# martinruenz/maskfusion

Hardware: NVIDIA H100
Metric: frames/sec on 640x480 .klg replay (higher is better)
Workload: dtype f32

## Files before the change

maskfusion_b200/csrc/mf_track.cu:

```cuda
#include "mf_common.cuh"
#include "mf_kernels.h"
#include "mf_host.h"
#include <float.h>
#include <algorithm>
#include <stdlib.h>
#include <string>

namespace mfb {

#ifndef MFB200_DEFAULT_TRACK_CACHE
#define MFB200_DEFAULT_TRACK_CACHE 0
#endif
#define CACHE_BYTES_PER_SLOT 44
#define TRK_THREADS 256
#define NACC_ICP 29
#define NACC_RGB 27
#define NACC (NACC_ICP + NACC_RGB)

MF_D float3 m3v(const float* R, float3 v)
{
    return make_float3((R[0] * v.x + R[1] * v.y) + R[2] * v.z, (R[3] * v.x + R[4] * v.y) + R[5] * v.z, (R[6] * v.x + R[7] * v.y) + R[8] * v.z);
}

__device__ void ldltSolve(const double* Ain, const double* b, int n, double* x)
// ... 245 lines not shown
{
    __shared__ bool isLast;
    __threadfence();
    __syncthreads();
    if (threadIdx.x == 0) {
        unsigned t = atomicAdd(ticket, 1u);
        isLast = (t == gridDim.x - 1);
        if (isLast) *ticket = 0;
    }
    __syncthreads();
    if (isLast) __threadfence();
    return isLast;
}

__global__ void __launch_bounds__(TRK_THREADS) k_icp_only(const float4* __restrict__ vmapC, const float4* __restrict__ nmapC,
                                                          const float4* __restrict__ vmapG, const float4* __restrict__ nmapG,
                                                          int W, int H, Cam cam, TrackPoses pp, float distThres, float angleThres,
                                                          double* __restrict__ partial, unsigned* ticket, float* out29)
{
    double acc[NACC_ICP];
#pragma unroll
    for (int k = 0; k < NACC_ICP; ++k) acc[k] = 0.0;
    const float* Rc = pp.p[0]; const float* tc = pp.p[0] + 9; const float* Rpi = pp.p[1]; const float* tp = pp.p[1] + 9;
    const float3 tprev = make_float3(tp[0], tp[1], tp[2]);
    const int N = W * H;
    for (int i = blockIdx.x * blockDim.x + threadIdx.x; i < N; i += gridDim.x * blockDim.x) {
        float4 vc4 = vmapC[i];
        float3 vg = m3v(Rc, make_float3(vc4.x, vc4.y, vc4.z));
        vg = make_float3(vg.x + tc[0], vg.y + tc[1], vg.z + tc[2]);
        float3 vcp = m3v(Rpi, sub3(vg, tprev));
        int ux = __float2int_rn(vcp.x * cam.fx / vcp.z + cam.cx);
        int uy = __float2int_rn(vcp.y * cam.fy / vcp.z + cam.cy);
        if (ux < 0 || uy < 0 || ux >= W || uy >= H || vcp.z < 0) continue;
        int j = uy * W + ux;
        float4 vp4 = __ldg(vmapG + j), np4 = __ldg(nmapG + j), nc4 = nmapC[i];
        float3 vp = make_float3(vp4.x, vp4.y, vp4.z), np_ = make_float3(np4.x, np4.y, np4.z);
        float3 ng = m3v(Rc, make_float3(nc4.x, nc4.y, nc4.z));
        float3 d = sub3(vp, vg);
        float dist = sqrtf((d.x * d.x + d.y * d.y) + d.z * d.z);
        float3 c = cross3(ng, np_);
        float sine = sqrtf((c.x * c.x + c.y * c.y) + c.z * c.z);
        if (!(sine < angleThres && dist <= distThres && !isnan(nc4.x) && !isnan(np4.x))) continue;
        float3 s_cp = vcp, d_cp = m3v(Rpi, sub3(vp, tprev)), n_cp = m3v(Rpi, np_);
        float row[7];
        row[0] = n_cp.x; row[1] = n_cp.y; row[2] = n_cp.z;
        row[3] = s_cp.y * n_cp.z - s_cp.z * n_cp.y;
        row[4] = s_cp.z * n_cp.x - s_cp.x * n_cp.z;
        row[5] = s_cp.x * n_cp.y - s_cp.y * n_cp.x;
        row[6] = (n_cp.x * (s_cp.x - d_cp.x) + n_cp.y * (s_cp.y - d_cp.y)) + n_cp.z * (s_cp.z - d_cp.z);
        int q = 0;
#pragma unroll
        for (int a = 0; a < 6; ++a)
#pragma unroll
            for (int b = a; b < 7; ++b) { acc[q] = fma((double)row[a], (double)row[b], acc[q]); ++q; }
        acc[27] = fma((double)row[6], (double)row[6], acc[27]);
        acc[28] += 1.0;
    }
    blockReduceStore<NACC_ICP>(acc, partial + (size_t)blockIdx.x * 32);
    if (!lastBlock(ticket)) return;
    __shared__ double tot[NACC_ICP];
    sumPartials<NACC_ICP>(partial, gridDim.x, tot);
    if (threadIdx.x < NACC_ICP) out29[threadIdx.x] = (float)tot[threadIdx.x];
}

#ifndef PT_THREADS
#define PT_THREADS 512
#endif
#define PT_WARPS (PT_THREADS / 32)
#define ROWF 32

struct TrackParams {
    int W, H; Cam cam;
    int icp, rgb, rgbOnly, so3;
    int iterations[3];
    float icpWeight, angleThres, distThres, sobelScale, maxDepthDelta;
    float minScale[3];
    int corrSlots;
    int bitWords;
    int cacheRounds;
    unsigned llBase;
    int nJobs; unsigned short jobStart[TRACK_MAX_JOBS + 1];
};

MF_D double shflXorD(double v, int m)
{
    return __hiloint2double(__shfl_xor_sync(0xffffffffu, __double2hiint(v), m), __shfl_xor_sync(0xffffffffu, __double2loint(v), m));
}
template <int H>
MF_D void warpHalvingStep(double* v, int lane)
{
    const bool up = (lane & H) != 0;
#pragma unroll
    for (int k = 0; k < H; ++k) {
        double keep = up ? v[k + H] : v[k];
        double send = up ? v[k] : v[k + H];
        v[k] = keep + shflXorD(send, H);
    }
}
MF_D void warpReduceHalving32(double* v)
{
    const int lane = threadIdx.x & 31;
    warpHalvingStep<16>(v, lane);
    warpHalvingStep<8>(v, lane);
    warpHalvingStep<4>(v, lane);
    warpHalvingStep<2>(v, lane);
    warpHalvingStep<1>(v, lane);
}

MF_D void llStore(uint4* p, double v, unsigned flag)
{
    asm volatile("st.volatile.global.v4.u32 [%0], {%1, %2, %3, %4};" ::"l"(p), "r"((unsigned)__double2loint(v)), "r"(flag), "r"((unsigned)__double2hiint(v)), "r"(flag) : "memory");
}
MF_D uint4 llLoad(const uint4* p)
{
    uint4 r;
    asm volatile("ld.volatile.global.v4.u32 {%0, %1, %2, %3}, [%4];" : "=r"(r.x), "=r"(r.y), "=r"(r.z), "=r"(r.w) : "l"(p) : "memory");
    return r;
}

template <int N>
MF_D void ctaReduceStore(const double* acc, double (*red)[ROWF], uint4* __restrict__ rowOut, unsigned flag, int extra0, int extra1)
{
    double v[32];
#pragma unroll
    for (int k = 0; k < 32; ++k) v[k] = k < N ? acc[k] : 0.0;
    v[29] = (double)extra0; v[30] = (double)extra1;
    warpReduceHalving32(v);
    const int lane = threadIdx.x & 31, warp = threadIdx.x >> 5;
    red[warp][lane] = v[0];
    __syncthreads();
    if (threadIdx.x < ROWF) {
        double s = 0;
#pragma unroll
        for (int w = 0; w < PT_WARPS; ++w) s += red[w][threadIdx.x];
        llStore(rowOut + threadIdx.x, s, flag);
    }
}
#define SUM_BATCH 10
MF_D void sumRows(const uint4* __restrict__ rows, unsigned R, unsigned flag, double (*ws)[ROWF], double* tot)
{
    const int lane = threadIdx.x & 31, warp = threadIdx.x >> 5;
    double a0 = 0;
    for (unsigned base = warp; base < R; base += PT_WARPS * SUM_BATCH) {
        uint4 x[SUM_BATCH];
        unsigned pending = 0;
#pragma unroll
        for (int i = 0; i < SUM_BATCH; ++i) { x[i] = make_uint4(0, 0, 0, 0); if (base + (unsigned)i * PT_WARPS < R) pending |= 1u << i; }
        while (pending) {
#pragma unroll
            for (int i = 0; i < SUM_BATCH; ++i)
                if ((pending >> i) & 1u) x[i] = llLoad(rows + (size_t)(base + (unsigned)i * PT_WARPS) * ROWF + lane);
#pragma unroll
            for (int i = 0; i < SUM_BATCH; ++i)
                if ((pending >> i) & 1u) { if (__all_sync(0xffffffffu, x[i].y == flag && x[i].w == flag)) pending &= ~(1u << i); }
        }
#pragma unroll
        for (int i = 0; i < SUM_BATCH; ++i) a0 += __hiloint2double((int)x[i].z, (int)x[i].x);
    }
    ws[warp][lane] = a0;
    __syncthreads();
    if (threadIdx.x < ROWF) {
        double s2 = 0;
#pragma unroll
        for (int w = 0; w < PT_WARPS; ++w) s2 += ws[w][threadIdx.x];
        tot[threadIdx.x] = s2;
    }
    __syncthreads();
}

struct RedCtx { uint4* rows; unsigned G, Gact, gen, llBase, bx; };
template <int N>
MF_D void reduceStep(const double* acc, int e0, int e1, bool active, RedCtx& rc, double (*red)[ROWF], double (*ws)[ROWF], double* tot)
{
    uint4* rows = rc.rows + (size_t)(rc.gen & 1) * rc.G * ROWF;
    ++rc.gen;
    const unsigned flag = rc.llBase + rc.gen;
    if (active) ctaReduceStore<N>(acc, red, rows + (size_t)rc.bx * ROWF, flag, e0, e1);
    sumRows(rows, rc.Gact, flag, ws, tot);
}

MF_D void gradU8(const uint8_t* __restrict__ img, int W, int x, int y, float& gx, float& gy)
{
    float actu = img[y * W + x], back = img[y * W + x - 1], fore = img[y * W + x + 1];
    gx = ((back + actu) / 2.0f) - ((fore + actu) / 2.0f);
    back = img[(y - 1) * W + x]; fore = img[(y + 1) * W + x];
    gy = ((back + actu) / 2.0f) - ((fore + actu) / 2.0f);
}


template <int LD>
MF_D double inv3dEntry(const double* M, int e)
{
    const int r = e / 3, c = e - 3 * r;
    const int c1 = c == 2 ? 0 : c + 1, c2 = c1 == 2 ? 0 : c1 + 1, r1 = r == 2 ? 0 : r + 1, r2 = r1 == 2 ? 0 : r1 + 1;
    const double cof = M[c1 * LD + r1] * M[c2 * LD + r2] - M[c1 * LD + r2] * M[c2 * LD + r1];
    const double c00 = M[LD + 1] * M[2 * LD + 2] - M[LD + 2] * M[2 * LD + 1], c01 = M[LD + 2] * M[2 * LD] - M[LD] * M[2 * LD + 2],
                 c02 = M[LD] * M[2 * LD + 1] - M[LD + 1] * M[2 * LD];
    const double det = M[0] * c00 + M[1] * c01 + M[2] * c02;
    return cof * (1.0 / det);
}

#ifdef MF_TRACK_TIMING
__device__ long long g_trackTiming[8192];
__device__ int g_trackTimingN;
#define TT(tag) do { if (blockIdx.x == 0 && threadIdx.x == 0) { int q_ = g_trackTimingN; if (q_ + 2 <= 8192) { g_trackTiming[q_] = (tag); g_trackTiming[q_ + 1] = clock64(); g_trackTimingN = q_ + 2; } } } while (0)
#else
#define TT(tag) do { } while (0)
#endif

struct SolveScratch { double A[36], b[6], x[6], Rt[16], nr[16], Ri[9], K[9], Kinv[9], tmp[9], ti[3]; float trR[9], trT[3], iR[9], iT[3]; int fast; };

MF_D void computeWarpCoop(TrackState* st, Cam c, SolveScratch* sc, int lane)
{
    const double* T = st->resultRt;
    const double* K = sc->K;
    if (lane < 9) sc->Ri[lane] = inv3dEntry<4>(T, lane);
    __syncwarp();
    if (lane < 3) sc->ti[lane] = -(sc->Ri[lane * 3] * T[3] + sc->Ri[lane * 3 + 1] * T[7] + sc->Ri[lane * 3 + 2] * T[11]);
    if (lane < 9) { int r = lane / 3, cc = lane % 3; sc->tmp[lane] = K[r * 3] * sc->Ri[cc] + K[r * 3 + 1] * sc->Ri[3 + cc] + K[r * 3 + 2] * sc->Ri[6 + cc]; }
    __syncwarp();
    if (lane < 9) { int r = lane / 3, cc = lane % 3; st->krk[lane] = (float)(sc->tmp[r * 3] * sc->Kinv[cc] + sc->tmp[r * 3 + 1] * sc->Kinv[3 + cc] + sc->tmp[r * 3 + 2] * sc->Kinv[6 + cc]); }
    if (lane < 3) st->kt[lane] = (float)(K[lane * 3] * sc->ti[0] + K[lane * 3 + 1] * sc->ti[1] + K[lane * 3 + 2] * sc->ti[2]);
    __syncwarp();
}

__device__ __noinline__ void solveAndUpdate(TrackState* st, const double* tot, bool ICP, bool RGB, float icpWeight, Cam cam, SolveScratch* sc)
{
    const int lane = threadIdx.x & 31;
    const double wgt = icpWeight;
    const int r6 = lane < 6 ? lane : 5;
    double arow[6], bown;
    {
        auto comb = [&](int c2, bool isA) -> double {
            const int a = r6 < c2 ? r6 : c2, b = r6 < c2 ? c2 : r6;
            const int q = 7 * a - (a * (a - 1)) / 2 + (b - a);
            const float vi = (float)tot[q], vr = (float)tot[NACC_ICP + q];
            if (ICP && RGB) return isA ? (double)vr + wgt * wgt * (double)vi : (double)vr + wgt * (double)vi;
            if (ICP) return (double)vi;
            return (double)vr;
        };
#pragma unroll
        for (int j = 0; j < 6; ++j) arow[j] = comb(j, true);
        bown = comb(6, false);
        if (lane < 6) {
#pragma unroll
            for (int j = 0; j < 6; ++j) st->lastA[lane * 6 + j] = arow[j];
            st->lastb[lane] = bown;
        }
    }
    if (ICP && lane == 31) { st->lastICPError = sqrtf((float)tot[27]) / (float)tot[28]; st->lastICPCount = (float)tot[28]; }
    TT(20);
    ldltSolvePivWarpRegs<6>(arow, bown, sc->x);
    TT(21);
    {
        double rx = sc->x[3], ry = sc->x[4], rz = sc->x[5];
        const double theta = sqrt(rx * rx + ry * ry + rz * rz);
        double c = 1.0, s = 0.0, c1 = 0.0;
        const bool rot = theta >= DBL_EPSILON;
        if (rot) { detSincos(theta, &s, &c); c1 = 1. - c; const double it = 1. / theta; rx *= it; ry *= it; rz *= it; }
        if (lane < 16) {
            const int r = lane >> 2, cc = lane & 3;
            double v;
            if (r == 3) v = cc == 3 ? 1.0 : 0.0;
            else if (cc == 3) v = sc->x[r];
            else if (!rot) v = r == cc ? 1.0 : 0.0;
            else {
                const double ur = r == 0 ? rx : r == 1 ? ry : rz, uc = cc == 0 ? rx : cc == 1 ? ry : rz;
                const double rrt = ur * uc;
                const int d = cc - r;
                const int o = 3 - r - cc;
                const double uo = o == 0 ? rx : o == 1 ? ry : rz;
                const double rxm = (r == cc) ? 0.0 : ((d == 1 || d == -2) ? -uo : uo);
                v = c * (r == cc ? 1.0 : 0.0) + c1 * rrt + s * rxm;
            }
            sc->Rt[lane] = v;
        }
    }
    __syncwarp();
    TT(22);
    if (lane < 16) {
        const int r = lane >> 2, c = lane & 3;
        double s2 = 0;
#pragma unroll
        for (int k = 0; k < 4; ++k) s2 += sc->Rt[r * 4 + k] * st->resultRt[k * 4 + c];
        sc->nr[lane] = s2;
    }
    __syncwarp();
    const double* T = sc->nr;
    if (lane < 16) st->resultRt[lane] = T[lane];
    if (lane < 9) st->trR[lane] = (float)T[(lane / 3) * 4 + lane % 3];
    else if (lane < 12) st->trT[lane - 9] = (float)T[(lane - 9) * 4 + 3];
    if (lane < 9) {
        const int r = lane / 3, c = lane % 3;
        const float i0 = (float)T[c * 4 + 0], i1 = (float)T[c * 4 + 1], i2 = (float)T[c * 4 + 2];
        st->Rcurr[lane] = (st->Rprev[r * 3] * i0 + st->Rprev[r * 3 + 1] * i1) + st->Rprev[r * 3 + 2] * i2;
    } else if (lane < 12) {
        const int r = lane - 9;
        const float t0 = (float)T[3], t1 = (float)T[7], t2 = (float)T[11];
        float iT[3];
#pragma unroll
        for (int k = 0; k < 3; ++k) iT[k] = -(((float)T[0 * 4 + k] * t0 + (float)T[1 * 4 + k] * t1) + (float)T[2 * 4 + k] * t2);
        st->tcurr[r] = ((st->Rprev[r * 3] * iT[0] + st->Rprev[r * 3 + 1] * iT[1]) + st->Rprev[r * 3 + 2] * iT[2]) + st->tprev[r];
    }
    TT(23);
    if (RGB && lane >= 16 && lane < 28) {
        const double* K = sc->K;
        double Ri[9];
#pragma unroll
        for (int e = 0; e < 9; ++e) Ri[e] = inv3dEntry<4>(T, e);
        const int l = lane - 16;
        if (l < 9) {
            const int r = l / 3, cc = l % 3;
            double tmp[3];
#pragma unroll
            for (int j = 0; j < 3; ++j) tmp[j] = K[r * 3] * Ri[j] + K[r * 3 + 1] * Ri[3 + j] + K[r * 3 + 2] * Ri[6 + j];
            st->krk[l] = (float)(tmp[0] * sc->Kinv[cc] + tmp[1] * sc->Kinv[3 + cc] + tmp[2] * sc->Kinv[6 + cc]);
        } else {
            const int q = l - 9;
            double ti[3];
#pragma unroll
            for (int j = 0; j < 3; ++j) ti[j] = -(Ri[j * 3] * T[3] + Ri[j * 3 + 1] * T[7] + Ri[j * 3 + 2] * T[11]);
            st->kt[q] = (float)(K[q * 3] * ti[0] + K[q * 3 + 1] * ti[1] + K[q * 3 + 2] * ti[2]);
        }
    }
}

MF_D void prefetchL1(const void* p) { asm volatile("prefetch.global.L1 [%0];" ::"l"(p)); }

struct PixA {
    float4 vc, nc; float d1; int valid, ni, x, y;
    bool rOK, iOK; int jr, ji, u0, v0; float td1; float3 vg, vcp;
    float d0; int li; float4 vp4, np4;
};

extern __shared__ int2 corrShared[];

__global__ void __launch_bounds__(PT_THREADS, 1) k_track_persistent(const TrackJob* __restrict__ jobs, TrackParams tp)
{
    __shared__ TrackJob J;
    __shared__ TrackState S;
    __shared__ SolveScratch sc;
    __shared__ double red[PT_WARPS][ROWF];
    __shared__ double ws[PT_WARPS][ROWF];
    __shared__ double tot[64];
    __shared__ double totR[ROWF];
    __shared__ float so3B[9], so3Kinv[9], so3Krlr[9];
    __shared__ double so3K[9], so3KinvD[9];
    __shared__ int flag;
    unsigned job = 0;
    while ((int)job + 1 < tp.nJobs && blockIdx.x >= tp.jobStart[job + 1]) ++job;
    const unsigned bx = blockIdx.x - tp.jobStart[job];
    const unsigned G = (unsigned)tp.jobStart[job + 1] - tp.jobStart[job];
    {
        const uint32_t* src = reinterpret_cast<const uint32_t*>(jobs + job);
        uint32_t* dst = reinterpret_cast<uint32_t*>(&J);
        for (int k = threadIdx.x; k < (int)(sizeof(TrackJob) / 4); k += PT_THREADS) dst[k] = src[k];
    }
    TrackState* st = &S;
#ifdef MF_TRACK_TIMING
    if (blockIdx.x == 0 && threadIdx.x == 0) g_trackTimingN = 0;
#endif
    TT(1);
    __syncthreads();
    if (threadIdx.x == 0) {
        const float* P = J.dpose->pose.m;
        for (int r = 0; r < 3; ++r) { for (int c = 0; c < 3; ++c) st->Rprev[r * 3 + c] = P[r * 4 + c]; st->tprev[r] = P[r * 4 + 3]; }
        for (int k = 0; k < 9; ++k) st->Rcurr[k] = st->Rprev[k];
        for (int k = 0; k < 3; ++k) st->tcurr[k] = st->tprev[k];
        inv3f(st->Rprev, st->RprevInv);
        for (int k = 0; k < 16; ++k) st->resultRt[k] = (k % 5 == 0) ? 1.0 : 0.0;
        for (int k = 0; k < 9; ++k) { st->resultR[k] = (k % 4 == 0) ? 1.0 : 0.0; st->lastResultR[k] = st->resultR[k]; st->R_lr[k] = (k % 4 == 0) ? 1.f : 0.f; st->trR[k] = (k % 4 == 0) ? 1.f : 0.f; }
        st->trT[0] = st->trT[1] = st->trT[2] = 0;
        st->so3LastError = FLT_MAX / 2; st->so3LastCount = FLT_MAX / 2; st->so3Done = 0;
        st->levelBreak = 0; st->lastRGBError = FLT_MAX; st->lastRGBCount = 0; st->lastICPError = 0; st->lastICPCount = 0;
        st->lastSO3Error = 0; st->lastSO3Count = 0; st->sigmaVal = 0;
        for (int k = 0; k < 36; ++k) st->lastA[k] = 0;
        for (int k = 0; k < 6; ++k) st->lastb[k] = 0;
    }
    __syncthreads();
    RedCtx rc;
    rc.rows = reinterpret_cast<uint4*>(J.partial); rc.G = G; rc.Gact = G; rc.gen = 0; rc.llBase = tp.llBase; rc.bx = bx;
    const size_t corrNeed = (size_t)((tp.W * tp.H + G * PT_THREADS - 1) / (G * PT_THREADS)) * PT_THREADS;
    int2* const corr = ((size_t)tp.corrSlots >= corrNeed && tp.corrSlots) ? corrShared : reinterpret_cast<int2*>(J.corres[0]) + (size_t)bx * corrNeed;
    const int cacheSlots = tp.cacheRounds * PT_THREADS;
    unsigned char* const cacheBase = reinterpret_cast<unsigned char*>(corrShared) + (((size_t)tp.corrSlots * sizeof(int2) + 15) & ~(size_t)15);
    float4* const vcS = reinterpret_cast<float4*>(cacheBase);
    float4* const ncS = vcS + cacheSlots;
    float* const d1S = reinterpret_cast<float*>(ncS + cacheSlots);
    uint32_t* const pkS = reinterpret_cast<uint32_t*>(d1S + cacheSlots);
    uint32_t* const gS = pkS + cacheSlots;
    uint32_t* const bitsS = gS + cacheSlots;

    if (tp.so3) {
        const int W = tp.W >> 2, H = tp.H >> 2, N = W * H;
        const unsigned Gact = min(G, (unsigned)((N + PT_THREADS - 1) / PT_THREADS));
        const bool active = bx < Gact;
        const int tid = (int)bx * PT_THREADS + threadIdx.x, nthr = (int)Gact * PT_THREADS;
        const Cam c = camLevel(tp.cam, 2);
        const uint8_t* __restrict__ lastImage = J.lastNextImage2;
        const uint8_t* __restrict__ nextImage = J.nextImage[2];
        if (threadIdx.x == 0) {
            double K[9] = {c.fx, 0, c.cx, 0, c.fy, c.cy, 0, 0, 1}, Kinv[9];
            inv3d(K, Kinv);
            for (int q = 0; q < 9; ++q) { so3K[q] = K[q]; so3KinvD[q] = Kinv[q]; so3Kinv[q] = (float)Kinv[q]; }
        }
        __syncthreads();
        for (int it = 0; it < 10; ++it) {
            if (threadIdx.x < 9) {
                const int r = threadIdx.x / 3, cc = threadIdx.x % 3;
                double kr[3];
#pragma unroll
                for (int q = 0; q < 3; ++q) kr[q] = so3K[r * 3] * st->resultR[q] + so3K[r * 3 + 1] * st->resultR[3 + q] + so3K[r * 3 + 2] * st->resultR[6 + q];
                so3Krlr[threadIdx.x] = (float)(cc == 0 ? kr[0] : cc == 1 ? kr[1] : kr[2]);
                so3B[threadIdx.x] = (float)(kr[0] * so3KinvD[cc] + kr[1] * so3KinvD[3 + cc] + kr[2] * so3KinvD[6 + cc]);
            }
            __syncthreads();
            TT(11);
            double acc[11];
#pragma unroll
            for (int k = 0; k < 11; ++k) acc[k] = 0;
            if (active) {
                for (int k = tid; k < N; k += nthr) {
                    int y = k / W, x = k - y * W;
                    float3 ur = make_float3((float)x, (float)y, 1.0f);
                    float3 wr = m3v(so3B, ur);
                    int wx = __float2int_rn(wr.x / wr.z), wy = __float2int_rn(wr.y / wr.z);
                    bool found = (wx >= 1 && wx < W - 1 && wy >= 1 && wy < H - 1 && x >= 1 && x < W - 1 && y >= 1 && y < H - 1);
                    if (found) {
                        float gnx, gny, glx, gly;
                        gradU8(nextImage, W, wx, wy, gnx, gny);
                        gradU8(lastImage, W, x, y, glx, gly);
                        float gx = (gnx + glx) / 2.0f, gy = (gny + gly) / 2.0f;
                        float3 p = m3v(so3Kinv, ur);
                        float z2 = p.z * p.z;
                        float a = so3Krlr[0], b = so3Krlr[1], cc = so3Krlr[2], d = so3Krlr[3], e = so3Krlr[4], f = so3Krlr[5], g = so3Krlr[6], h = so3Krlr[7], i = so3Krlr[8];
                        float fy = (float)y, fxx = (float)x;
                        float3 l = make_float3(((p.z * (d * gy + a * gx)) - (gy * g * fy) - (gx * g * fxx)) / z2,
                                               ((p.z * (e * gy + b * gx)) - (gy * h * fy) - (gx * h * fxx)) / z2,
                                               ((p.z * (f * gy + cc * gx)) - (gy * i * fy) - (gx * i * fxx)) / z2);
                        float row[4];
                        row[0] = l.y * p.z - l.z * p.y;
                        row[1] = l.z * p.x - l.x * p.z;
                        row[2] = l.x * p.y - l.y * p.x;
                        row[3] = -((float)nextImage[wy * W + wx] - (float)lastImage[k]);
                        int q = 0;
#pragma unroll
                        for (int ii = 0; ii < 3; ++ii)
#pragma unroll
                            for (int jj = ii; jj < 4; ++jj) { acc[q] = fma((double)row[ii], (double)row[jj], acc[q]); ++q; }
                        acc[9] = fma((double)row[3], (double)row[3], acc[9]);
                        acc[10] += 1.0;
                    }
                }
            }
            TT(12);
            rc.Gact = Gact;
            reduceStep<11>(acc, 0, 0, active, rc, red, ws, tot);
            TT(15);
            if (threadIdx.x < 32) {
                int mode = 0;
                if (threadIdx.x == 0) {
                    float res0 = (float)tot[9], res1 = (float)tot[10];
                    st->lastSO3Error = sqrtf(res0) / res1; st->lastSO3Count = res1;
                    if (st->lastSO3Error < st->so3LastError && fabsf(st->so3LastError - st->lastSO3Count) < 0.001f) mode = 0;
                    else if (st->lastSO3Error > st->so3LastError + 0.001f) {
                        st->lastSO3Error = st->so3LastError; st->lastSO3Count = st->so3LastCount;
                        for (int q = 0; q < 9; ++q) st->resultR[q] = st->lastResultR[q];
                        mode = 1;
                    } else {
                        st->so3LastError = st->lastSO3Error; st->so3LastCount = st->lastSO3Count;
                        for (int q = 0; q < 9; ++q) st->lastResultR[q] = st->resultR[q];
                        double* A = sc.A; double* bb = sc.b;
                        A[0] = (double)(float)tot[0]; A[1] = A[3] = (double)(float)tot[1]; A[2] = A[6] = (double)(float)tot[2]; bb[0] = (double)(float)tot[3];
                        A[4] = (double)(float)tot[4]; A[5] = A[7] = (double)(float)tot[5]; bb[1] = (double)(float)tot[6];
                        A[8] = (double)(float)tot[7]; bb[2] = (double)(float)tot[8];
                        mode = 2;
                    }
                }
                mode = __shfl_sync(0xffffffffu, mode, 0);
                if (mode == 2) {
                    __syncwarp();
                    ldltSolvePivWarp<3>(sc.A, sc.b, sc.x);
                    if (threadIdx.x == 0) {
                        double delta[3];
                        for (int k = 0; k < 3; ++k) delta[k] = (double)(float)sc.x[k];
                        double ru[9]; rodrigues(delta, ru);
                        float ruf[9], n[9];
                        for (int k = 0; k < 9; ++k) ruf[k] = (float)ru[k];
                        for (int r = 0; r < 3; ++r) for (int cc2 = 0; cc2 < 3; ++cc2) n[r * 3 + cc2] = (ruf[r * 3] * st->R_lr[cc2] + ruf[r * 3 + 1] * st->R_lr[3 + cc2]) + ruf[r * 3 + 2] * st->R_lr[6 + cc2];
                        for (int k = 0; k < 9; ++k) { st->R_lr[k] = n[k]; st->resultR[k] = n[k]; }
                    }
                }
                if (threadIdx.x == 0) flag = mode != 2;
            }
            TT(16);
            __syncthreads();
            if (flag) break;
        }
        __syncthreads();
        if (threadIdx.x == 0)
            for (int r = 0; r < 3; ++r) for (int cc = 0; cc < 3; ++cc) st->resultRt[r * 4 + cc] = st->resultR[r * 3 + cc];
        __syncthreads();
    }

    for (int level = 2; level >= 0; --level) {
        if (tp.iterations[level] == 0) continue;
        const int W = tp.W >> level, H = tp.H >> level, N = W * H;
        const unsigned Gact = min(G, (unsigned)((N + PT_THREADS - 1) / PT_THREADS));
        const bool active = bx < Gact;
        const int tid = (int)bx * PT_THREADS + threadIdx.x, nthr = (int)Gact * PT_THREADS;
        const int fullRounds = N / nthr;
        int kTail = -1;
        if (active) {
            const int j = (threadIdx.x >> 5) * (int)Gact + (int)bx;
            const int kt = fullRounds * nthr + j * 32 + (threadIdx.x & 31);
            if (kt < N) kTail = kt;
        }
        const int rounds = active ? fullRounds + (kTail >= 0 ? 1 : 0) : 0;
        auto kOf = [&](int r) { return r < fullRounds ? tid + r * nthr : kTail; };
        const Cam cam = camLevel(tp.cam, level);
        const float4* __restrict__ vmapC = J.vmapC[level];
        const float4* __restrict__ nmapC = J.nmapC[level];
        const float4* __restrict__ vmapG = J.vmapG[level];
        const float4* __restrict__ nmapG = J.nmapG[level];
        const float4* __restrict__ cloud = J.cloud[level];
        const short2* __restrict__ grad = J.nextGrad[level];
        const float* __restrict__ lastDepth = J.lastDepth[level];
        const float* __restrict__ nextDepth = J.lastDepth[level];
        const uint8_t* __restrict__ lastImage = J.lastImage[level];
        const uint8_t* __restrict__ nextImage = J.nextImage[level];
        const uint8_t* __restrict__ rgbValid = J.rgbValid[level];
        if (threadIdx.x < 32) {
            if (threadIdx.x == 0) { st->levelBreak = 0; st->lastRGBError = FLT_MAX; }
            if (threadIdx.x < 9) {
                const int r = threadIdx.x / 3, cc = threadIdx.x % 3;
                sc.K[threadIdx.x] = r == cc ? (r == 0 ? (double)cam.fx : r == 1 ? (double)cam.fy : 1.0) : (cc == 2 ? (r == 0 ? (double)cam.cx : (double)cam.cy) : 0.0);
            }
            __syncwarp();
            if (threadIdx.x < 9) sc.Kinv[threadIdx.x] = inv3dEntry<3>(sc.K, threadIdx.x);
            __syncwarp();
            if (tp.rgb) computeWarpCoop(st, cam, &sc, threadIdx.x);
        }
        __syncthreads();

        const bool useBits = tp.icp && tp.bitWords > 0 && J.validBits[level] != nullptr && (N + 31) / 32 <= tp.bitWords;
        if (useBits) {
            const uint32_t* __restrict__ src = J.validBits[level];
            for (int k = threadIdx.x; k < (N + 31) / 32; k += PT_THREADS) bitsS[k] = __ldg(src + k);
        }
        __syncthreads();
        const int cRounds = min(rounds, tp.cacheRounds);
        for (int r = 0; r < cRounds; ++r) {
            const int k = kOf(r), slot = r * PT_THREADS + threadIdx.x;
            const int y = k / W, x = k - y * W;
            uint32_t pk = ((uint32_t)x << 9) | ((uint32_t)y << 20);
            float d1 = 0.f; float4 vc = make_float4(0, 0, 0, 0), nc = vc; uint32_t g = 0;
            if (tp.rgb) { pk |= (rgbValid[k] ? 1u : 0u) | ((uint32_t)nextImage[k] << 1); d1 = nextDepth[k]; const short2 gg = grad[k]; g = (uint32_t)(uint16_t)gg.x | ((uint32_t)(uint16_t)gg.y << 16); }
            if (tp.icp) { vc = vmapC[k]; nc = nmapC[k]; }
            vcS[slot] = vc; ncS[slot] = nc; d1S[slot] = d1; pkS[slot] = pk; gS[slot] = g;
        }
        auto stage0 = [&](PixA& p, int k, int r) {
            if (r < cRounds) {
                const int slot = r * PT_THREADS + threadIdx.x;
                const uint32_t pk = pkS[slot];
                p.valid = (int)(pk & 1u); p.ni = (int)((pk >> 1) & 0xffu); p.x = (int)((pk >> 9) & 0x7ffu); p.y = (int)(pk >> 20);
                p.d1 = d1S[slot]; p.vc = vcS[slot]; p.nc = ncS[slot];
                return;
            }
            p.valid = 0; p.d1 = 0.f; p.ni = 0; p.vc = make_float4(0, 0, 0, 0); p.nc = p.vc;
            p.y = k / W; p.x = k - p.y * W;
            if (tp.rgb) { p.valid = rgbValid[k]; p.d1 = nextDepth[k]; p.ni = nextImage[k]; }
            if (tp.icp) { p.vc = vmapC[k]; p.nc = nmapC[k]; }
        };
        auto stage1 = [&](PixA& p, int k, const float3 tprev) {
            p.rOK = false; p.iOK = false; p.jr = 0; p.ji = 0; p.u0 = 0; p.v0 = 0; p.td1 = 0.f;
            p.vg = make_float3(0, 0, 0); p.vcp = p.vg;
            const int y = p.y, x = p.x;
            if (tp.rgb && p.valid && !isnan(p.d1)) {
                const float* K = st->krk; const float* kt = st->kt;
                const float d1 = p.d1;
                p.td1 = d1 * ((K[6] * x + K[7] * y) + K[8]) + kt[2];
                float fu = (d1 * ((K[0] * x + K[1] * y) + K[2]) + kt[0]) / p.td1;
                float fv = (d1 * ((K[3] * x + K[4] * y) + K[5]) + kt[1]) / p.td1;
                p.u0 = (fu != fu || fabsf(fu) > 1e9f) ? -1 : __float2int_rn(fu);
                p.v0 = (fv != fv || fabsf(fv) > 1e9f) ? -1 : __float2int_rn(fv);
                if (p.u0 >= 0 && p.v0 >= 0 && p.u0 < W && p.v0 < H) { p.rOK = true; p.jr = p.v0 * W + p.u0; }
            }
            if (tp.icp) {
                float3 vg = m3v(st->Rcurr, make_float3(p.vc.x, p.vc.y, p.vc.z));
                vg = make_float3(vg.x + st->tcurr[0], vg.y + st->tcurr[1], vg.z + st->tcurr[2]);
                float3 vcp = m3v(st->RprevInv, sub3(vg, tprev));
                int ux = __float2int_rn(vcp.x * cam.fx / vcp.z + cam.cx);
                int uy = __float2int_rn(vcp.y * cam.fy / vcp.z + cam.cy);
                if (!(ux < 0 || uy < 0 || ux >= W || uy >= H || vcp.z < 0)) {
                    p.ji = uy * W + ux;
                    p.iOK = !useBits || ((bitsS[p.ji >> 5] >> (p.ji & 31)) & 1u);
                }
                p.vg = vg; p.vcp = vcp;
            }
        };
        auto stage2 = [&](PixA& p) {
            p.d0 = 0.f; p.li = 0; p.vp4 = make_float4(0, 0, 0, 0); p.np4 = p.vp4;
            if (p.rOK) { p.d0 = lastDepth[p.jr]; p.li = lastImage[p.jr]; }
            if (p.iOK) { p.vp4 = __ldg(vmapG + p.ji); p.np4 = __ldg(nmapG + p.ji); }
        };

        for (int it = 0; it < tp.iterations[level]; ++it) {
            TT(100 + level);
            double acc[NACC_ICP];
#pragma unroll
            for (int k = 0; k < NACC_ICP; ++k) acc[k] = 0.0;
            int cnt = 0, sig = 0;
            if (active) {
                const float3 tprev = make_float3(st->tprev[0], st->tprev[1], st->tprev[2]);
                auto stage3 = [&](const PixA& p, int k, int slot) {
                    if (tp.rgb) {
                        int2 c = make_int2(-1, 0);
                        if (p.rOK && p.d0 > 0 && fabsf(p.td1 - p.d0) <= tp.maxDepthDelta && p.li != 0) {
                            const float diff = (float)p.ni - (float)p.li;
                            c.x = (p.u0 & 0xffff) | (p.v0 << 16); c.y = __float_as_int(diff);
                            cnt += 1;
                            sig += (int)(diff * diff);
                        }
                        corr[slot] = c;
                    }
                    if (p.iOK) {
                        const float4 nc4 = p.nc, vp4 = p.vp4, np4 = p.np4;
                        float3 vp = make_float3(vp4.x, vp4.y, vp4.z), np_ = make_float3(np4.x, np4.y, np4.z);
                        float3 ng = m3v(st->Rcurr, make_float3(nc4.x, nc4.y, nc4.z));
                        float3 d = sub3(vp, p.vg);
                        float dist = sqrtf((d.x * d.x + d.y * d.y) + d.z * d.z);
                        float3 c = cross3(ng, np_);
                        float sine = sqrtf((c.x * c.x + c.y * c.y) + c.z * c.z);
                        bool found = (sine < tp.angleThres && dist <= tp.distThres && !isnan(nc4.x) && !isnan(np4.x));
                        if (found) {
                            float3 s_cp = p.vcp;
                            float3 d_cp = m3v(st->RprevInv, sub3(vp, tprev));
                            float3 n_cp = m3v(st->RprevInv, np_);
                            float row[7];
                            row[0] = n_cp.x; row[1] = n_cp.y; row[2] = n_cp.z;
                            row[3] = s_cp.y * n_cp.z - s_cp.z * n_cp.y;
                            row[4] = s_cp.z * n_cp.x - s_cp.x * n_cp.z;
                            row[5] = s_cp.x * n_cp.y - s_cp.y * n_cp.x;
                            row[6] = (n_cp.x * (s_cp.x - d_cp.x) + n_cp.y * (s_cp.y - d_cp.y)) + n_cp.z * (s_cp.z - d_cp.z);
                            int q = 0;
#pragma unroll
                            for (int a = 0; a < 6; ++a)
#pragma unroll
                                for (int b = a; b < 7; ++b) { acc[q] = fma((double)row[a], (double)row[b], acc[q]); ++q; }
                            acc[27] = fma((double)row[6], (double)row[6], acc[27]);
                            acc[28] += 1.0;
                        }
                    }
                };
                for (int r = 0; r < rounds; r += 2) {
                    const bool two = r + 1 < rounds;
                    const int k0 = kOf(r), k1 = two ? kOf(r + 1) : k0;
                    for (int q = 2; q < 4; ++q)
                        if (r + q < rounds && r + q >= cRounds) {
                            const int kn = kOf(r + q);
                            if (tp.icp) { prefetchL1(vmapC + kn); prefetchL1(nmapC + kn); }
                            if (tp.rgb) { prefetchL1(nextDepth + kn); }
                        }
                    PixA a, b;
                    stage0(a, k0, r);
                    if (two) stage0(b, k1, r + 1); else { b.valid = 0; b.d1 = 0.f; b.ni = 0; b.x = 0; b.y = 0; b.vc = make_float4(0, 0, 0, 0); b.nc = b.vc; }
                    stage1(a, k0, tprev);
                    if (two) stage1(b, k1, tprev); else { b.rOK = false; b.iOK = false; b.jr = 0; b.ji = 0; b.u0 = 0; b.v0 = 0; b.td1 = 0.f; b.vg = make_float3(0, 0, 0); b.vcp = b.vg; }
                    stage2(a); stage2(b);
                    stage3(a, k0, r * PT_THREADS + threadIdx.x);
                    if (two) stage3(b, k1, (r + 1) * PT_THREADS + threadIdx.x);
                }
            }
            TT(2);
            rc.Gact = Gact;
            if (tp.rgb && rounds > cRounds) { prefetchL1(grad + kOf(cRounds)); }
            reduceStep<NACC_ICP>(acc, cnt, sig, active, rc, red, ws, tot);
            TT(5);
            if (tp.rgb) {
                if (threadIdx.x == 0) {
                    int rgbSize = (int)(long long)tot[29], sigma = (int)(long long)tot[30];
                    float tmpError = (float)(sqrt((double)sigma) / (double)rgbSize);
                    float sigmaVal = (tmpError == 0) ? 1 : (float)rgbSize;
                    int brk = 0;
                    if (tp.rgbOnly && tmpError > st->lastRGBError) brk = 1;
                    else {
                        st->lastRGBError = tmpError; st->lastRGBCount = (float)rgbSize;
                        if (tp.rgbOnly) sigmaVal = -1;
                        st->sigmaVal = sigmaVal;
                    }
                    flag = brk;
                }
                __syncthreads();
                if (flag) break;
                double accR[NACC_RGB];
#pragma unroll
                for (int k = 0; k < NACC_RGB; ++k) accR[k] = 0.0;
                if (active) {
                    const float sigmaSh = st->sigmaVal;
                    auto rgbRow = [&](int2 c, short2 g, float4 cp) {
                        const float diff = __int_as_float(c.y);
                        float w = sigmaSh + fabsf(diff);
                        w = w > 1.19209290E-07F ? 1.0f / w : 1.0f;
                        if (sigmaSh == -1) w = 1;
                        float row[7];
                        row[6] = -w * diff;
                        const float invz = cp.w;
                        float dIdx_v = w * tp.sobelScale * (float)g.x;
                        float dIdy_v = w * tp.sobelScale * (float)g.y;
                        float v0 = dIdx_v * cam.fx * invz;
                        float v1 = dIdy_v * cam.fy * invz;
                        float v2 = -(v0 * cp.x + v1 * cp.y) * invz;
                        row[0] = v0; row[1] = v1; row[2] = v2;
                        row[3] = -cp.z * v1 + cp.y * v2;
                        row[4] = cp.z * v0 - cp.x * v2;
                        row[5] = -cp.y * v0 + cp.x * v1;
                        int q = 0;
#pragma unroll
                        for (int a = 0; a < 6; ++a)
#pragma unroll
                            for (int b = a; b < 7; ++b) { accR[q] = fma((double)row[a], (double)row[b], accR[q]); ++q; }
                    };
                    for (int r = 0; r < rounds; r += 2) {
                        const bool two = r + 1 < rounds;
                        const int k0 = kOf(r), k1 = two ? kOf(r + 1) : k0;
                        const int2 c0 = corr[r * PT_THREADS + threadIdx.x];
                        const int2 c1 = two ? corr[(r + 1) * PT_THREADS + threadIdx.x] : make_int2(-1, 0);
                        short2 g0 = make_short2(0, 0), g1 = g0;
                        float4 p0 = make_float4(0, 0, 1, 0), p1 = p0;
                        auto gradOf = [&](int k, int rr) -> short2 {
                            if (rr < cRounds) { const uint32_t g = gS[rr * PT_THREADS + threadIdx.x]; return make_short2((short)(g & 0xffffu), (short)(g >> 16)); }
                            return grad[k];
                        };
                        if (c0.x != -1) { g0 = gradOf(k0, r); p0 = cloud[(c0.x >> 16) * W + (c0.x & 0xffff)]; }
                        if (c1.x != -1) { g1 = gradOf(k1, r + 1); p1 = cloud[(c1.x >> 16) * W + (c1.x & 0xffff)]; }
                        if (c0.x != -1) rgbRow(c0, g0, p0);
                        if (c1.x != -1) rgbRow(c1, g1, p1);
                    }
                }
                TT(6);
                for (int q = cRounds; q < cRounds + 2; ++q)
                    if (q < rounds) {
                        const int kn = kOf(q);
                        if (tp.icp) { prefetchL1(vmapC + kn); prefetchL1(nmapC + kn); }
                        prefetchL1(nextDepth + kn);
                    }
                reduceStep<NACC_RGB>(accR, 0, 0, active, rc, red, ws, totR);
                TT(9);
                if (threadIdx.x < NACC_RGB) tot[NACC_ICP + threadIdx.x] = totR[threadIdx.x];
                __syncthreads();
            }
            if (threadIdx.x < 32) solveAndUpdate(st, tot, tp.icp != 0, tp.rgb != 0, tp.icpWeight, cam, &sc);
            __syncthreads();
            TT(10);
        }
        __syncthreads();
    }

    TT(99);
    if (bx == 0 && threadIdx.x == 0) {
        float dx = st->tcurr[0] - st->tprev[0], dy = st->tcurr[1] - st->tprev[1], dz = st->tcurr[2] - st->tprev[2];
        if (tp.rgb && sqrtf((dx * dx + dy * dy) + dz * dz) > 0.3f) {
            for (int k = 0; k < 9; ++k) { st->Rcurr[k] = st->Rprev[k]; st->trR[k] = (k % 4 == 0) ? 1.f : 0.f; }
            for (int k = 0; k < 3; ++k) { st->tcurr[k] = st->tprev[k]; st->trT[k] = 0; }
        }
        float* po = st->out;
        for (int k = 0; k < 32; ++k) po[k] = ((k % 16) % 5 == 0) ? 1.f : 0.f;
        for (int r = 0; r < 3; ++r) {
            for (int c = 0; c < 3; ++c) { po[r * 4 + c] = st->Rcurr[r * 3 + c]; po[16 + r * 4 + c] = st->trR[r * 3 + c]; }
            po[r * 4 + 3] = st->tcurr[r]; po[16 + r * 4 + 3] = st->trT[r];
        }
        po[32] = st->lastICPError; po[33] = st->lastICPCount; po[34] = st->lastRGBError; po[35] = st->lastRGBCount;
        po[36] = st->lastSO3Error; po[37] = st->lastSO3Count;
        *J.st = *st;
        float last[16];
        for (int k = 0; k < 16; ++k) last[k] = (k % 5 == 0) ? 1.f : 0.f;
        for (int r = 0; r < 3; ++r) { for (int c = 0; c < 3; ++c) last[r * 4 + c] = st->Rprev[r * 3 + c]; last[r * 4 + 3] = st->tprev[r]; }
        derivePose(J.dpose, po, last);
    }
}

float track_min_scale(int level)
{
    const float minGrad[3] = {5, 3, 1};
    const float sobelScale = (float)(1.0 / 8.0);
    return (float)(pow((double)minGrad[level], 2.0) / pow((double)sobelScale, 2.0));
}

static int trackBlocks(int N, int numSMs)
{
    int need = (N + TRK_THREADS - 1) / TRK_THREADS;
    int cap = numSMs * 2;
    if (cap > TRACK_MAX_BLOCKS) cap = TRACK_MAX_BLOCKS;
    return need < cap ? need : cap;
}

void track_shares(int nJobs, unsigned lightMask, int totalCTAs, int ratio, int* G)
{
    if (nJobs < 1) return;
    int Geq = totalCTAs / nJobs;
    if (Geq > TRACK_MAX_BLOCKS / 2) Geq = TRACK_MAX_BLOCKS / 2;
    int nLight = 0;
    for (int j = 0; j < nJobs; ++j) nLight += (lightMask >> j) & 1u;
    const int nHeavy = nJobs - nLight;
    int Gheavy = Geq, Glight = Geq;
    if (nLight > 0 && nHeavy > 0) {
        Glight = std::max(4, totalCTAs / (nLight + std::max(1, ratio) * nHeavy));
        Gheavy = (totalCTAs - nLight * Glight) / nHeavy;
        if (Gheavy < Glight) { Gheavy = Geq; Glight = Geq; }
        if (Gheavy > TRACK_MAX_BLOCKS / 2) Gheavy = TRACK_MAX_BLOCKS / 2;
    }
    for (int j = 0; j < nJobs; ++j) G[j] = ((lightMask >> j) & 1u) ? Glight : Gheavy;
}

int launch_tracking(TrackJob* d_jobs, int nJobs, int W, int H, Cam cam, bool rgbOnly, float icpWeight,
                    bool pyramid, bool fastOdom, bool so3, int numSMs, cudaStream_t s, unsigned lightMask)
{
    const bool anyValidBits = lightMask != 0;
    static int coResidentDev[64]; static size_t dynMaxDev[64]; static bool devInit[64];
    int dev = 0; cudaCheck(cudaGetDevice(&dev), "cudaGetDevice");
    if (dev < 0 || dev >= 64) throw CudaError{"device ordinal above 63"};
    if (!devInit[dev]) {
        int perSM = 0;
        cudaError_t e = cudaOccupancyMaxActiveBlocksPerMultiprocessor(&perSM, k_track_persistent, PT_THREADS, 0);
        if (e != cudaSuccess || perSM < 1) throw CudaError{std::string("k_track_persistent does not fit on an SM: ") + cudaGetErrorString(e)};
        coResidentDev[dev] = perSM * numSMs;
        int optin = 0; cudaDeviceGetAttribute(&optin, cudaDevAttrMaxSharedMemoryPerBlockOptin, dev);
        cudaFuncAttributes fa; cudaCheck(cudaFuncGetAttributes(&fa, k_track_persistent), "cudaFuncGetAttributes");
        dynMaxDev[dev] = (size_t)optin > fa.sharedSizeBytes + 2048 ? (size_t)optin - fa.sharedSizeBytes - 2048 : 0;
        cudaCheck(cudaFuncSetAttribute(k_track_persistent, cudaFuncAttributeMaxDynamicSharedMemorySize, (int)dynMaxDev[dev]), "cudaFuncSetAttribute");
// ... 70 lines not shown
```

Before: 729.2.

## Accumulate normal-equation outer products with FP64 MMA tensor core instructions

Each thread now writes its Jacobian row (plus residual and count column) into a per-warp shared tile instead of keeping per-thread double accumulators for the upper triangle. A warp then forms J^T J with mma.m8n8k4 f64, giving a 2-double fragment per lane. The CTA reduction is rewritten to read the needed fragment entries by index, which drops the shuffle-halving reduction of 29 doubles. Loops are made warp-uniform (roundsW, k<N guard) so the collective MMA is legal. The cost is extra shared-memory traffic and __syncwarp per pair of pixels, and float-to-double conversion of row values before the MMA.

```diff
diff --git a/maskfusion_b200/csrc/mf_track.cu b/maskfusion_b200/csrc/mf_track.cu
--- a/maskfusion_b200/csrc/mf_track.cu
+++ b/maskfusion_b200/csrc/mf_track.cu
@@ -351,29 +351,40 @@
     int nJobs; unsigned short jobStart[TRACK_MAX_JOBS + 1];
 };
 
-MF_D double shflXorD(double v, int m)
-{
-    return __hiloint2double(__shfl_xor_sync(0xffffffffu, __double2hiint(v), m), __shfl_xor_sync(0xffffffffu, __double2loint(v), m));
-}
-template <int H>
-MF_D void warpHalvingStep(double* v, int lane)
-{
-    const bool up = (lane & H) != 0;
-#pragma unroll
-    for (int k = 0; k < H; ++k) {
-        double keep = up ? v[k + H] : v[k];
-        double send = up ? v[k] : v[k + H];
-        v[k] = keep + shflXorD(send, H);
-    }
-}
-MF_D void warpReduceHalving32(double* v)
-{
+union WarpScratch {
+    float rows[2][32][8];
+    double frag[66];
+};
+
+MF_D void putRow(float* slot, float4 lo, float4 hi)
+{
+    reinterpret_cast<float4*>(slot)[0] = lo;
+    reinterpret_cast<float4*>(slot)[1] = hi;
+}
+
+MF_D void warpAccumulate(float (*tile)[8], bool has, double (&f)[2])
+{
+    if (!__any_sync(0xffffffffu, has)) return;
     const int lane = threadIdx.x & 31;
-    warpHalvingStep<16>(v, lane);
-    warpHalvingStep<8>(v, lane);
-    warpHalvingStep<4>(v, lane);
-    warpHalvingStep<2>(v, lane);
-    warpHalvingStep<1>(v, lane);
+    if (!has) putRow(tile[lane], make_float4(0.f, 0.f, 0.f, 0.f), make_float4(0.f, 0.f, 0.f, 0.f));
+    __syncwarp();
+#pragma unroll
+    for (int i = 0; i < 8; ++i) {
+        const double v = (double)tile[4 * i + (lane & 3)][lane >> 2];
+        asm("mma.sync.aligned.m8n8k4.row.col.f64.f64.f64.f64 {%0, %1}, {%2}, {%3}, {%0, %1};" : "+d"(f[0]), "+d"(f[1]) : "d"(v), "d"(v));
+    }
+    __syncwarp();
+}
+
+template <int R>
+MF_D int fragIndex(int q)
+{
+    constexpr int nJ = R * (R + 1) / 2 - 1;
+    if (q == nJ) return (R - 1) * 9;
+    if (q == nJ + 1) return R * 9;
+    int a = 0;
+    while (q >= R - a) { q -= R - a; ++a; }
+    return a * 9 + q;
 }
 
 MF_D void llStore(uint4* p, double v, unsigned flag)
@@ -387,22 +398,23 @@
     return r;
 }
 
-template <int N>
-MF_D void ctaReduceStore(const double* acc, double (*red)[ROWF], uint4* __restrict__ rowOut, unsigned flag, int extra0, int extra1)
-{
-    double v[32];
-#pragma unroll
-    for (int k = 0; k < 32; ++k) v[k] = k < N ? acc[k] : 0.0;
-    v[29] = (double)extra0; v[30] = (double)extra1;
-    warpReduceHalving32(v);
+template <int R, int N>
+MF_D void ctaReduceStore(const double (&f)[2], WarpScratch* wsc, uint4* __restrict__ rowOut, unsigned flag, int extra0, int extra1)
+{
     const int lane = threadIdx.x & 31, warp = threadIdx.x >> 5;
-    red[warp][lane] = v[0];
+    const int c0 = __reduce_add_sync(0xffffffffu, extra0), c1 = __reduce_add_sync(0xffffffffu, extra1);
+    reinterpret_cast<double2*>(wsc[warp].frag)[lane] = make_double2(f[0], f[1]);
+    if (lane == 0) { wsc[warp].frag[64] = (double)c0; wsc[warp].frag[65] = (double)c1; }
     __syncthreads();
     if (threadIdx.x < ROWF) {
+        const int q = threadIdx.x;
+        const int e = q < N ? fragIndex<R>(q) : (q == 29 || q == 30) ? 64 + (q - 29) : -1;
         double s = 0;
-#pragma unroll
-        for (int w = 0; w < PT_WARPS; ++w) s += red[w][threadIdx.x];
-        llStore(rowOut + threadIdx.x, s, flag);
+        if (e >= 0) {
+#pragma unroll
+            for (int w = 0; w < PT_WARPS; ++w) s += wsc[w].frag[e];
+        }
+        llStore(rowOut + q, s, flag);
     }
 }
 #define SUM_BATCH 10
@@ -438,13 +450,13 @@
 }
 
 struct RedCtx { uint4* rows; unsigned G, Gact, gen, llBase, bx; };
-template <int N>
-MF_D void reduceStep(const double* acc, int e0, int e1, bool active, RedCtx& rc, double (*red)[ROWF], double (*ws)[ROWF], double* tot)
+template <int R, int N>
+MF_D void reduceStep(const double (&f)[2], int e0, int e1, bool active, RedCtx& rc, WarpScratch* wsc, double (*ws)[ROWF], double* tot)
 {
     uint4* rows = rc.rows + (size_t)(rc.gen & 1) * rc.G * ROWF;
     ++rc.gen;
     const unsigned flag = rc.llBase + rc.gen;
-    if (active) ctaReduceStore<N>(acc, red, rows + (size_t)rc.bx * ROWF, flag, e0, e1);
+    if (active) ctaReduceStore<R, N>(f, wsc, rows + (size_t)rc.bx * ROWF, flag, e0, e1);
     sumRows(rows, rc.Gact, flag, ws, tot);
 }
 
@@ -609,7 +621,7 @@
     __shared__ TrackJob J;
     __shared__ TrackState S;
     __shared__ SolveScratch sc;
-    __shared__ double red[PT_WARPS][ROWF];
+    __shared__ __align__(16) WarpScratch wsc[PT_WARPS];
     __shared__ double ws[PT_WARPS][ROWF];
     __shared__ double tot[64];
     __shared__ double totR[ROWF];
@@ -685,16 +697,15 @@
             }
             __syncthreads();
             TT(11);
-            double acc[11];
-#pragma unroll
-            for (int k = 0; k < 11; ++k) acc[k] = 0;
+            double f[2] = {0.0, 0.0};
             if (active) {
-                for (int k = tid; k < N; k += nthr) {
+                for (int k0 = tid - (threadIdx.x & 31); k0 < N; k0 += nthr) {
+                    const int k = k0 + (threadIdx.x & 31);
                     int y = k / W, x = k - y * W;
                     float3 ur = make_float3((float)x, (float)y, 1.0f);
                     float3 wr = m3v(so3B, ur);
                     int wx = __float2int_rn(wr.x / wr.z), wy = __float2int_rn(wr.y / wr.z);
-                    bool found = (wx >= 1 && wx < W - 1 && wy >= 1 && wy < H - 1 && x >= 1 && x < W - 1 && y >= 1 && y < H - 1);
+                    bool found = (k < N && wx >= 1 && wx < W - 1 && wy >= 1 && wy < H - 1 && x >= 1 && x < W - 1 && y >= 1 && y < H - 1);
                     if (found) {
                         float gnx, gny, glx, gly;
                         gradU8(nextImage, W, wx, wy, gnx, gny);
@@ -707,24 +718,16 @@
                         float3 l = make_float3(((p.z * (d * gy + a * gx)) - (gy * g * fy) - (gx * g * fxx)) / z2,
                                                ((p.z * (e * gy + b * gx)) - (gy * h * fy) - (gx * h * fxx)) / z2,
                                                ((p.z * (f * gy + cc * gx)) - (gy * i * fy) - (gx * i * fxx)) / z2);
-                        float row[4];
-                        row[0] = l.y * p.z - l.z * p.y;
-                        row[1] = l.z * p.x - l.x * p.z;
-                        row[2] = l.x * p.y - l.y * p.x;
-                        row[3] = -((float)nextImage[wy * W + wx] - (float)lastImage[k]);
-                        int q = 0;
-#pragma unroll
-                        for (int ii = 0; ii < 3; ++ii)
-#pragma unroll
-                            for (int jj = ii; jj < 4; ++jj) { acc[q] = fma((double)row[ii], (double)row[jj], acc[q]); ++q; }
-                        acc[9] = fma((double)row[3], (double)row[3], acc[9]);
-                        acc[10] += 1.0;
+                        putRow(wsc[threadIdx.x >> 5].rows[0][threadIdx.x & 31],
+                               make_float4(l.y * p.z - l.z * p.y, l.z * p.x - l.x * p.z, l.x * p.y - l.y * p.x, -((float)nextImage[wy * W + wx] - (float)lastImage[k])),
+                               make_float4(1.f, 0.f, 0.f, 0.f));
                     }
+                    warpAccumulate(wsc[threadIdx.x >> 5].rows[0], found, f);
                 }
             }
             TT(12);
             rc.Gact = Gact;
-            reduceStep<11>(acc, 0, 0, active, rc, red, ws, tot);
+            reduceStep<4, 11>(f, 0, 0, active, rc, wsc, ws, tot);
             TT(15);
             if (threadIdx.x < 32) {
                 int mode = 0;
@@ -786,7 +789,10 @@
             if (kt < N) kTail = kt;
         }
         const int rounds = active ? fullRounds + (kTail >= 0 ? 1 : 0) : 0;
+        const bool tailW = __any_sync(0xffffffffu, kTail >= 0);
+        const int roundsW = active ? fullRounds + (tailW ? 1 : 0) : 0;
         auto kOf = [&](int r) { return r < fullRounds ? tid + r * nthr : kTail; };
+        float (*const tiles)[32][8] = wsc[threadIdx.x >> 5].rows;
         const Cam cam = camLevel(tp.cam, level);
         const float4* __restrict__ vmapC = J.vmapC[level];
         const float4* __restrict__ nmapC = J.nmapC[level];
@@ -841,6 +847,7 @@
             if (tp.rgb) { p.valid = rgbValid[k]; p.d1 = nextDepth[k]; p.ni = nextImage[k]; }
             if (tp.icp) { p.vc = vmapC[k]; p.nc = nmapC[k]; }
         };
+        auto noPixel0 = [&](PixA& p) { p.valid = 0; p.d1 = 0.f; p.ni = 0; p.x = 0; p.y = 0; p.vc = make_float4(0, 0, 0, 0); p.nc = p.vc; };
         auto stage1 = [&](PixA& p, int k, const float3 tprev) {
             p.rOK = false; p.iOK = false; p.jr = 0; p.ji = 0; p.u0 = 0; p.v0 = 0; p.td1 = 0.f;
             p.vg = make_float3(0, 0, 0); p.vcp = p.vg;
@@ -868,6 +875,7 @@
                 p.vg = vg; p.vcp = vcp;
             }
         };
+        auto noPixel1 = [&](PixA& p) { p.rOK = false; p.iOK = false; p.jr = 0; p.ji = 0; p.u0 = 0; p.v0 = 0; p.td1 = 0.f; p.vg = make_float3(0, 0, 0); p.vcp = p.vg; };
         auto stage2 = [&](PixA& p) {
             p.d0 = 0.f; p.li = 0; p.vp4 = make_float4(0, 0, 0, 0); p.np4 = p.vp4;
             if (p.rOK) { p.d0 = lastDepth[p.jr]; p.li = lastImage[p.jr]; }
@@ -876,13 +884,11 @@
 
         for (int it = 0; it < tp.iterations[level]; ++it) {
             TT(100 + level);
-            double acc[NACC_ICP];
-#pragma unroll
-            for (int k = 0; k < NACC_ICP; ++k) acc[k] = 0.0;
+            double f[2] = {0.0, 0.0};
             int cnt = 0, sig = 0;
             if (active) {
                 const float3 tprev = make_float3(st->tprev[0], st->tprev[1], st->tprev[2]);
-                auto stage3 = [&](const PixA& p, int k, int slot) {
+                auto stage3 = [&](const PixA& p, int slot, float* row) -> bool {
                     if (tp.rgb) {
                         int2 c = make_int2(-1, 0);
                         if (p.rOK && p.d0 > 0 && fabsf(p.td1 - p.d0) <= tp.maxDepthDelta && p.li != 0) {
@@ -906,25 +912,17 @@
                             float3 s_cp = p.vcp;
                             float3 d_cp = m3v(st->RprevInv, sub3(vp, tprev));
                             float3 n_cp = m3v(st->RprevInv, np_);
-                            float row[7];
-                            row[0] = n_cp.x; row[1] = n_cp.y; row[2] = n_cp.z;
-                            row[3] = s_cp.y * n_cp.z - s_cp.z * n_cp.y;
-                            row[4] = s_cp.z * n_cp.x - s_cp.x * n_cp.z;
-                            row[5] = s_cp.x * n_cp.y - s_cp.y * n_cp.x;
-                            row[6] = (n_cp.x * (s_cp.x - d_cp.x) + n_cp.y * (s_cp.y - d_cp.y)) + n_cp.z * (s_cp.z - d_cp.z);
-                            int q = 0;
-#pragma unroll
-                            for (int a = 0; a < 6; ++a)
-#pragma unroll
-                                for (int b = a; b < 7; ++b) { acc[q] = fma((double)row[a], (double)row[b], acc[q]); ++q; }
-                            acc[27] = fma((double)row[6], (double)row[6], acc[27]);
-                            acc[28] += 1.0;
+                            putRow(row, make_float4(n_cp.x, n_cp.y, n_cp.z, s_cp.y * n_cp.z - s_cp.z * n_cp.y),
+                                   make_float4(s_cp.z * n_cp.x - s_cp.x * n_cp.z, s_cp.x * n_cp.y - s_cp.y * n_cp.x,
+                                               (n_cp.x * (s_cp.x - d_cp.x) + n_cp.y * (s_cp.y - d_cp.y)) + n_cp.z * (s_cp.z - d_cp.z), 1.f));
+                            return true;
                         }
                     }
+                    return false;
                 };
-                for (int r = 0; r < rounds; r += 2) {
-                    const bool two = r + 1 < rounds;
-                    const int k0 = kOf(r), k1 = two ? kOf(r + 1) : k0;
+                for (int r = 0; r < roundsW; r += 2) {
+                    const bool hasA = r < rounds, hasB = r + 1 < rounds;
+                    const int k0 = hasA ? kOf(r) : 0, k1 = hasB ? kOf(r + 1) : k0;
                     for (int q = 2; q < 4; ++q)
                         if (r + q < rounds && r + q >= cRounds) {
                             const int kn = kOf(r + q);
@@ -932,19 +930,21 @@
                             if (tp.rgb) { prefetchL1(nextDepth + kn); }
                         }
                     PixA a, b;
-                    stage0(a, k0, r);
-                    if (two) stage0(b, k1, r + 1); else { b.valid = 0; b.d1 = 0.f; b.ni = 0; b.x = 0; b.y = 0; b.vc = make_float4(0, 0, 0, 0); b.nc = b.vc; }
-                    stage1(a, k0, tprev);
-                    if (two) stage1(b, k1, tprev); else { b.rOK = false; b.iOK = false; b.jr = 0; b.ji = 0; b.u0 = 0; b.v0 = 0; b.td1 = 0.f; b.vg = make_float3(0, 0, 0); b.vcp = b.vg; }
+                    if (hasA) stage0(a, k0, r); else noPixel0(a);
+                    if (hasB) stage0(b, k1, r + 1); else noPixel0(b);
+                    if (hasA) stage1(a, k0, tprev); else noPixel1(a);
+                    if (hasB) stage1(b, k1, tprev); else noPixel1(b);
                     stage2(a); stage2(b);
-                    stage3(a, k0, r * PT_THREADS + threadIdx.x);
-                    if (two) stage3(b, k1, (r + 1) * PT_THREADS + threadIdx.x);
+                    const bool fA = hasA && stage3(a, r * PT_THREADS + threadIdx.x, tiles[0][threadIdx.x & 31]);
+                    const bool fB = hasB && stage3(b, (r + 1) * PT_THREADS + threadIdx.x, tiles[1][threadIdx.x & 31]);
+                    warpAccumulate(tiles[0], fA, f);
+                    warpAccumulate(tiles[1], fB, f);
                 }
             }
             TT(2);
             rc.Gact = Gact;
             if (tp.rgb && rounds > cRounds) { prefetchL1(grad + kOf(cRounds)); }
-            reduceStep<NACC_ICP>(acc, cnt, sig, active, rc, red, ws, tot);
+            reduceStep<7, NACC_ICP>(f, cnt, sig, active, rc, wsc, ws, tot);
             TT(5);
             if (tp.rgb) {
                 if (threadIdx.x == 0) {
@@ -962,39 +962,27 @@
                 }
                 __syncthreads();
                 if (flag) break;
-                double accR[NACC_RGB];
-#pragma unroll
-                for (int k = 0; k < NACC_RGB; ++k) accR[k] = 0.0;
+                double fR[2] = {0.0, 0.0};
                 if (active) {
                     const float sigmaSh = st->sigmaVal;
-                    auto rgbRow = [&](int2 c, short2 g, float4 cp) {
+                    auto rgbRow = [&](int2 c, short2 g, float4 cp, float* row) {
                         const float diff = __int_as_float(c.y);
                         float w = sigmaSh + fabsf(diff);
                         w = w > 1.19209290E-07F ? 1.0f / w : 1.0f;
                         if (sigmaSh == -1) w = 1;
-                        float row[7];
-                        row[6] = -w * diff;
                         const float invz = cp.w;
                         float dIdx_v = w * tp.sobelScale * (float)g.x;
                         float dIdy_v = w * tp.sobelScale * (float)g.y;
                         float v0 = dIdx_v * cam.fx * invz;
                         float v1 = dIdy_v * cam.fy * invz;
                         float v2 = -(v0 * cp.x + v1 * cp.y) * invz;
-                        row[0] = v0; row[1] = v1; row[2] = v2;
-                        row[3] = -cp.z * v1 + cp.y * v2;
-                        row[4] = cp.z * v0 - cp.x * v2;
-                        row[5] = -cp.y * v0 + cp.x * v1;
-                        int q = 0;
-#pragma unroll
-                        for (int a = 0; a < 6; ++a)
-#pragma unroll
-                            for (int b = a; b < 7; ++b) { accR[q] = fma((double)row[a], (double)row[b], accR[q]); ++q; }
+                        putRow(row, make_float4(v0, v1, v2, -cp.z * v1 + cp.y * v2), make_float4(cp.z * v0 - cp.x * v2, -cp.y * v0 + cp.x * v1, -w * diff, 0.f));
                     };
-                    for (int r = 0; r < rounds; r += 2) {
-                        const bool two = r + 1 < rounds;
-                        const int k0 = kOf(r), k1 = two ? kOf(r + 1) : k0;
-                        const int2 c0 = corr[r * PT_THREADS + threadIdx.x];
-                        const int2 c1 = two ? corr[(r + 1) * PT_THREADS + threadIdx.x] : make_int2(-1, 0);
+                    for (int r = 0; r < roundsW; r += 2) {
+                        const bool hasA = r < rounds, hasB = r + 1 < rounds;
+                        const int k0 = hasA ? kOf(r) : 0, k1 = hasB ? kOf(r + 1) : k0;
+                        const int2 c0 = hasA ? corr[r * PT_THREADS + threadIdx.x] : make_int2(-1, 0);
+                        const int2 c1 = hasB ? corr[(r + 1) * PT_THREADS + threadIdx.x] : make_int2(-1, 0);
                         short2 g0 = make_short2(0, 0), g1 = g0;
                         float4 p0 = make_float4(0, 0, 1, 0), p1 = p0;
                         auto gradOf = [&](int k, int rr) -> short2 {
@@ -1003,8 +991,10 @@
                         };
                         if (c0.x != -1) { g0 = gradOf(k0, r); p0 = cloud[(c0.x >> 16) * W + (c0.x & 0xffff)]; }
                         if (c1.x != -1) { g1 = gradOf(k1, r + 1); p1 = cloud[(c1.x >> 16) * W + (c1.x & 0xffff)]; }
-                        if (c0.x != -1) rgbRow(c0, g0, p0);
-                        if (c1.x != -1) rgbRow(c1, g1, p1);
+                        if (c0.x != -1) rgbRow(c0, g0, p0, tiles[0][threadIdx.x & 31]);
+                        if (c1.x != -1) rgbRow(c1, g1, p1, tiles[1][threadIdx.x & 31]);
+                        warpAccumulate(tiles[0], c0.x != -1, fR);
+                        warpAccumulate(tiles[1], c1.x != -1, fR);
                     }
                 }
                 TT(6);
@@ -1014,7 +1004,7 @@
                         if (tp.icp) { prefetchL1(vmapC + kn); prefetchL1(nmapC + kn); }
                         prefetchL1(nextDepth + kn);
                     }
-                reduceStep<NACC_RGB>(accR, 0, 0, active, rc, red, ws, totR);
+                reduceStep<7, NACC_RGB>(fR, 0, 0, active, rc, wsc, ws, totR);
                 TT(9);
                 if (threadIdx.x < NACC_RGB) tot[NACC_ICP + threadIdx.x] = totR[threadIdx.x];
                 __syncthreads();
```

After: 755.4, median of 6. 1.04x the previous value.
